# c976237222/HunyuanVideo_efficiency

Hardware: AMD Instinct MI355X
Metric: denoise-steps/sec (720x1280x129f, HunyuanVideo DiT 20+40 blocks, bf16) (higher is better)
Workload: dtype bf16

## Files before the change

hunyuanvideo_efficiency_amd/csrc/hv_attention.hip:

```cpp
#include "hv_attention.hpp"

using namespace hv_attn;

namespace {

constexpr int QTILE = 256;

__global__ __launch_bounds__(256) void attn_combine_kernel(const float* __restrict__ part_o, const float* __restrict__ part_ml,
                                                            bf16_t* __restrict__ o, int64_t so, int n_q, int n_heads, int n_splits) {
    const int64_t idx = (int64_t)blockIdx.x * blockDim.x + threadIdx.x;
    const int64_t total = (int64_t)n_q * n_heads * 32;
    if (idx >= total) return;
    const int d4 = (int)(idx & 31);
    const int64_t rh = idx >> 5;
    const int head = (int)(rh % n_heads);
    const int64_t row = rh / n_heads;
    float m = -INFINITY;
    for (int s = 0; s < n_splits; ++s) m = fmaxf(m, part_ml[(((int64_t)s * n_q + row) * n_heads + head) * 2]);
    float4 acc = make_float4(0.f, 0.f, 0.f, 0.f);
    float l = 0.f;
    for (int s = 0; s < n_splits; ++s) {
        const int64_t ri = ((int64_t)s * n_q + row) * n_heads + head;
        const float w = __builtin_amdgcn_exp2f(part_ml[ri * 2] - m);
        const float4 v = *reinterpret_cast<const float4*>(part_o + ri * D + d4 * 4);
        acc.x += v.x * w; acc.y += v.y * w; acc.z += v.z * w; acc.w += v.w * w;
        l += part_ml[ri * 2 + 1] * w;
    }
    const float inv = 1.0f / l;
    u32x2 w2;
    w2[0] = pack_bf2(acc.x * inv, acc.y * inv);
    w2[1] = pack_bf2(acc.z * inv, acc.w * inv);
    *reinterpret_cast<u32x2*>(o + row * so + head * D + d4 * 4) = w2;
}

int attn_launch(const AttnArgs& a, dim3 grid, hipStream_t stream) { return launch_w4(a, grid, stream); }

constexpr int KMAX_ROWS = 2048;
__global__ __launch_bounds__(256) void attn_kmax_kernel(const bf16_t* __restrict__ k, int64_t sk, int n_kv, unsigned* __restrict__ out) {
    __shared__ float wmax[4];
    const int head = blockIdx.y, t = threadIdx.x, ch = t & 15;
    const int r0 = blockIdx.x * KMAX_ROWS, r1 = min(r0 + KMAX_ROWS, n_kv);
    float best = 0.f;
    for (int row = r0 + (t >> 4); row < r1; row += 16) {
        const u32x4 w = *reinterpret_cast<const u32x4*>(k + (int64_t)row * sk + head * D + ch * 8);
        float s = 0.f;
#pragma unroll
        for (int j = 0; j < 4; ++j) {
            const float lo = bf2f_lo(w[j]), hi = bf2f_hi(w[j]);
            s += lo * lo + hi * hi;
        }
#pragma unroll
        for (int o = 8; o > 0; o >>= 1) s += __shfl_xor(s, o, 64);
        best = fmaxf(best, s);
    }
    best = fmaxf(best, __shfl_xor(best, 16, 64));
    best = fmaxf(best, __shfl_xor(best, 32, 64));
    if ((t & 63) == 0) wmax[t >> 6] = best;
    __syncthreads();
    if (t == 0) atomicMax(out + head, __float_as_uint(fmaxf(fmaxf(wmax[0], wmax[1]), fmaxf(wmax[2], wmax[3]))));
}

int attn_prepare_kmax(AttnArgs& a, void* workspace, int64_t workspace_bytes, hipStream_t stream) {
    a.kmax2 = nullptr;
    if (!workspace || workspace_bytes < KMAX_BYTES || a.n_heads > KMAX_HEADS || a.n_kv < 64 * KVT) return HV_OK;
    if (hipMemsetAsync(workspace, 0, KMAX_BYTES, stream) != hipSuccess) return HV_ERR_LAUNCH;
    attn_kmax_kernel<<<dim3((unsigned)((a.n_kv + KMAX_ROWS - 1) / KMAX_ROWS), (unsigned)a.n_heads), dim3(256), 0, stream>>>(a.k, a.sk, a.n_kv, (unsigned*)workspace);
    a.kmax2 = (const unsigned*)workspace;
    return HV_OK;
}

}

extern "C" int64_t hv_attn_workspace_bytes(int n_q, int n_kv, int n_heads) {
    (void)n_kv;
    return (int64_t)KMAX_BYTES + (int64_t)2 * n_q * n_heads * (128 + 2) * (int64_t)sizeof(float);
}

extern "C" int hv_attn_fwd_bf16(const void* q, const void* k, const void* v, void* o, int64_t stride_q, int64_t stride_k,
                                int64_t stride_v, int64_t stride_o, int n_q, int n_kv, int n_heads, int head_dim,
                                float scale, void* workspace, int64_t workspace_bytes, hipStream_t stream) {
    if (!q || !k || !v || !o || head_dim != D || n_heads <= 0 || n_q < 0 || n_kv < 0 || (stride_q & 7) || (stride_k & 7) ||
        (stride_v & 7) || (stride_o & 3))
        return HV_ERR_ARG;
    if (n_q == 0) return HV_OK;
    if (n_kv == 0) return HV_ERR_ARG;
    AttnArgs a;
    a.q = (const bf16_t*)q; a.k = (const bf16_t*)k; a.v = (const bf16_t*)v; a.o = (bf16_t*)o;
    a.sq = stride_q; a.sk = stride_k; a.sv = stride_v; a.so = stride_o;
    a.n_q = n_q; a.n_kv = n_kv; a.n_heads = n_heads;
    a.n_qtiles = (n_q + QTILE - 1) / QTILE;
    a.scale_log2e = scale * 1.4426950408889634f;
    a.n_splits = 1; a.split_keys = n_kv; a.part_o = nullptr; a.part_ml = nullptr; a.partial = 0;
    if (attn_prepare_kmax(a, workspace, workspace_bytes, stream) != HV_OK) return HV_ERR_LAUNCH;
    {
        const int64_t nwg = (int64_t)a.n_qtiles * n_heads;
        const int ntile = (n_kv + KVT - 1) / KVT;
        const double r1 = (double)((nwg + 255) / 256), r2 = 0.5 * (double)((2 * nwg + 255) / 256);
        if (workspace && ntile >= 64 && r2 < 0.97 * r1 && workspace_bytes >= hv_attn_workspace_bytes(n_q, n_kv, n_heads)) {
            a.n_splits = 2;
            a.split_keys = ((ntile + 1) / 2) * KVT;
            a.part_o = (float*)((char*)workspace + KMAX_BYTES);
            a.part_ml = a.part_o + (int64_t)2 * n_q * n_heads * D;
        }
    }
    if (attn_launch(a, dim3((unsigned)(a.n_qtiles * n_heads), (unsigned)a.n_splits), stream) != HV_OK) return HV_ERR_LAUNCH;
    if (a.n_splits > 1) {
        const int64_t total = (int64_t)n_q * n_heads * 32;
        attn_combine_kernel<<<dim3((unsigned)((total + 255) / 256)), dim3(256), 0, stream>>>(a.part_o, a.part_ml, a.o, a.so, n_q, n_heads,
                                                                                           a.n_splits);
    }
    return hv_check_launch();
}

extern "C" int hv_attn_partial_bf16(const void* q, const void* k, const void* v, int64_t stride_q, int64_t stride_k, int64_t stride_v,
                                    int n_q, int n_kv, int n_heads, int head_dim, float scale, void* part_o, void* part_ml,
                                    int n_slots, int slot, int splits, hipStream_t stream) {
    if (!q || !k || !v || !part_o || !part_ml || head_dim != D || n_heads <= 0 || n_q < 0 || n_kv <= 0 || (stride_q & 7) ||
        (stride_k & 7) || (stride_v & 7) || (splits != 1 && splits != 2) || slot < 0 || slot + splits > n_slots)
        return HV_ERR_ARG;
    if (n_q == 0) return HV_OK;
    const int ntile = (n_kv + KVT - 1) / KVT;
    if (splits == 2 && ntile < 2) return HV_ERR_ARG;
    AttnArgs a;
    a.q = (const bf16_t*)q; a.k = (const bf16_t*)k; a.v = (const bf16_t*)v; a.o = nullptr;
    a.sq = stride_q; a.sk = stride_k; a.sv = stride_v; a.so = 0;
    a.n_q = n_q; a.n_kv = n_kv; a.n_heads = n_heads;
    a.n_qtiles = (n_q + QTILE - 1) / QTILE;
    a.scale_log2e = scale * 1.4426950408889634f;
    a.n_splits = splits;
    a.split_keys = splits == 2 ? ((ntile + 1) / 2) * KVT : n_kv;
    a.part_o = (float*)part_o + (int64_t)slot * n_q * n_heads * D;
    a.part_ml = (float*)part_ml + (int64_t)slot * n_q * n_heads * 2;
    a.partial = 1;
    a.kmax2 = nullptr;
    if (attn_launch(a, dim3((unsigned)(a.n_qtiles * n_heads), (unsigned)splits), stream) != HV_OK) return HV_ERR_LAUNCH;
    return hv_check_launch();
}

extern "C" int hv_attn_merge_bf16(const void* part_o, const void* part_ml, void* o, int64_t stride_o, int n_q, int n_heads, int n_slots,
                                  hipStream_t stream) {
    if (!part_o || !part_ml || !o || n_heads <= 0 || n_q < 0 || n_slots <= 0 || (stride_o & 3)) return HV_ERR_ARG;
    if (n_q == 0) return HV_OK;
    const int64_t total = (int64_t)n_q * n_heads * 32;
    attn_combine_kernel<<<dim3((unsigned)((total + 255) / 256)), dim3(256), 0, stream>>>((const float*)part_o, (const float*)part_ml,
                                                                                       (bf16_t*)o, stride_o, n_q, n_heads, n_slots);
    return hv_check_launch();
}

extern "C" int hv_attn_suggest_splits(int n_q, int n_kv, int n_heads) {
    const int64_t nwg = (int64_t)((n_q + QTILE - 1) / QTILE) * n_heads;
    const int ntile = (n_kv + KVT - 1) / KVT;
    const double r1 = (double)((nwg + 255) / 256), r2 = 0.5 * (double)((2 * nwg + 255) / 256);
    return (ntile >= 64 && r2 < 0.97 * r1) ? 2 : 1;
}
```

hunyuanvideo_efficiency_amd/ops.py:

```python
from __future__ import annotations

from typing import Optional

import torch

from . import _lib

BF16 = torch.bfloat16
ACT_NONE, ACT_GELU_TANH, ACT_SILU = 0, 1, 2
PROFILE_ATTN = None


def _chk(t: torch.Tensor, dtype, name: str, last_contig: bool = True):
    if not t.is_cuda:
        raise _lib.HVKernelError(f"{name}: expected a GPU tensor (this package has no CPU path), got {t.device}")
    if t.dtype != dtype:
        raise TypeError(f"{name}: expected {dtype}, got {t.dtype}")
    if last_contig and t.dim() > 0 and t.stride(-1) != 1:
        raise ValueError(f"{name}: innermost dimension must be contiguous")


def _rows(t: torch.Tensor, name: str):
    if t.dim() == 1:
        return 1, t.shape[0], t.shape[0]
    d = t.shape[-1]
    n = t.numel() // d
    ld = t.stride(-2)
    exp = ld
    for i in range(t.dim() - 2, -1, -1):
        if t.shape[i] != 1 and t.stride(i) != exp:
            raise ValueError(f"{name}: rows are not uniformly strided {t.shape} {t.stride()}")
        exp *= t.shape[i]
    return n, d, ld


def ln_modulate(x, shift=None, scale=None, out=None, eps: float = 1e-6, affine: bool = False):
    _chk(x, BF16, "x")
    m, d, ldx = _rows(x, "x")
    if out is None:
        out = torch.empty(x.shape, dtype=BF16, device=x.device)
    _chk(out, BF16, "out")
    mo, do, ldo = _rows(out, "out")
    assert (mo, do) == (m, d)
    for t, n in ((shift, "shift"), (scale, "scale")):
        if t is not None:
            _chk(t, BF16, n)
            assert t.numel() == d and t.is_contiguous(), f"{n} must be a contiguous [{d}] vector (batch 1)"
    _lib.call("ln_modulate_bf16", x, shift, scale, out, m, d, ldx, ldo, eps,
                                               1 if affine else 0)
    return out


def qknorm_rope_(qkv, q_weight, k_weight, cos, sin, n_rope: int, n_heads: int, k_offset: int, eps: float = 1e-6, out=None):
    _chk(qkv, BF16, "qkv")
    n, _, ld = _rows(qkv, "qkv")
    _chk(q_weight, BF16, "q_weight"), _chk(k_weight, BF16, "k_weight")
    if n_rope > 0:
        _chk(cos, torch.float32, "cos"), _chk(sin, torch.float32, "sin")
        assert cos.is_contiguous() and sin.is_contiguous() and cos.shape[-1] == 128 and cos.shape[0] >= n_rope
    if out is not None:
        _chk(out, BF16, "out", False)
        assert out.dim() == 3 and out.shape[0] == n and out.stride(2) == 1 and out.shape[2] % 128 == 0
        assert out.shape[1] * out.shape[2] == 2 * n_heads * 128, (out.shape, n_heads)
        _lib.call("qknorm_rope_scatter_bf16", qkv, q_weight, k_weight, cos, sin, n, n_rope, n_heads, 128, ld, k_offset, eps,
                  out, out.stride(0), out.shape[2] // 128, out.stride(1))
        return out
    _lib.call("qknorm_rope_bf16", qkv, q_weight, k_weight, cos, sin, n,
                                               n_rope, n_heads, 128, ld, k_offset, eps)
    return qkv


def gemm(a, w, bias=None, out=None, act: int = ACT_NONE, n_split: int = 0, out1=None, act1: int = ACT_NONE,
         gate=None, res=None):
    _chk(a, BF16, "a"), _chk(w, BF16, "w")
    m, k, lda = _rows(a, "a")
    n, kw, ldw = _rows(w, "w")
    assert k == kw, (a.shape, w.shape)
    n0 = n_split if 0 < n_split < n else n
    if out is None:
        out = torch.empty(*a.shape[:-1], n0, dtype=BF16, device=a.device)
    _chk(out, BF16, "out")
    mo, no, ld0 = _rows(out, "out")
    assert mo == m and no >= n0
    ld1 = 0
    if n0 < n:
        _chk(out1, BF16, "out1")
        m1, n1, ld1 = _rows(out1, "out1")
        assert m1 == m and n1 >= n - n0
    for t, nm in ((bias, "bias"), (gate, "gate")):
        if t is not None:
            _chk(t, BF16, nm)
            assert t.numel() == n and t.is_contiguous()
    ld_res = 0
    if res is not None:
        _chk(res, BF16, "res")
        mr, nr, ld_res = _rows(res, "res")
        assert mr == m and nr == n
    _lib.call("gemm_bf16", a, lda, w, ldw, bias, m, n, k, out, ld0, act, n0,
                                        out1, ld1, act1, gate, res, ld_res)
    return out


def linear_smallm(x, w, bias=None, silu_in: bool = False, silu_out: bool = False, out=None, addend=None):
    _chk(x, BF16, "x"), _chk(w, BF16, "w")
    m, k, ldx = _rows(x, "x")
    n, kw, ldw = _rows(w, "w")
    assert k == kw and ldw == k and m <= 4
    if out is None:
        out = torch.empty(*x.shape[:-1], n, dtype=BF16, device=x.device)
    _, _, ldo = _rows(out, "out")
    if bias is not None:
        _chk(bias, BF16, "bias")
    if addend is not None:
        _chk(addend, BF16, "addend")
        assert addend.shape == out.shape and addend.stride() == out.stride()
    _lib.call("linear_smallm_bf16", x, w, bias, addend, out, m, n, k, ldx, ldo,
                                                 (1 if silu_in else 0) | (2 if silu_out else 0))
    return out


_attn_ws = {}


ATTN_MIN_WORKSPACE = 256


def _attn_workspace(n_q, n_kv, n_heads, device):
    if n_kv < 64 * 64:
        return None
    n_wg = ((n_q + 255) // 256) * n_heads
    need = ATTN_MIN_WORKSPACE if n_wg >= 16 * 256 else int(_lib.host("attn_workspace_bytes", n_q, n_kv, n_heads))
    key = str(device)
    ws = _attn_ws.get(key)
    if ws is None or ws.numel() < need:
        ws = torch.empty(need, dtype=torch.uint8, device=device)
        _attn_ws[key] = ws
    return ws


def attn_fwd(q, k, v, out, n_heads: int, scale: Optional[float] = None, kv_split_workspace: bool = True):
    for t, nm in ((q, "q"), (k, "k"), (v, "v"), (out, "out")):
        _chk(t, BF16, nm)
        assert t.dim() == 2
    n_q, n_kv = q.shape[0], k.shape[0]
    assert v.shape[0] == n_kv and out.shape[0] == n_q
    if scale is None:
        scale = 128 ** -0.5
    prof = PROFILE_ATTN
    if prof is not None:
        e0, e1 = torch.cuda.Event(enable_timing=True), torch.cuda.Event(enable_timing=True)
        e0.record()
    ws = _attn_workspace(n_q, n_kv, n_heads, q.device) if kv_split_workspace else None
    _lib.call("attn_fwd_bf16", q, k, v, out, q.stride(0), k.stride(0), v.stride(0),
                                            out.stride(0), n_q, n_kv, n_heads, 128, scale, ws,
                                            0 if ws is None else ws.numel())
    if prof is not None:
        e1.record()
        prof.append((e0, e1, n_q, n_kv, n_heads))
    return out


class AttnPartials:

    def __init__(self, n_slots: int, n_q: int, n_heads: int, device):
        self.n_slots, self.n_q, self.n_heads = n_slots, n_q, n_heads
        self.o = torch.empty(n_slots, n_q, n_heads, 128, dtype=torch.float32, device=device)
        self.ml = torch.empty(n_slots, n_q, n_heads, 2, dtype=torch.float32, device=device)
        self.used = 0


def attn_suggest_splits(n_q: int, n_kv: int, n_heads: int) -> int:
    return int(_lib.host("attn_suggest_splits", n_q, n_kv, n_heads))


def attn_partial(q, k, v, parts: AttnPartials, n_heads: int, splits: int = 1, scale: Optional[float] = None):
    for t, nm in ((q, "q"), (k, "k"), (v, "v")):
        _chk(t, BF16, nm)
        assert t.dim() == 2
    n_q, n_kv = q.shape[0], k.shape[0]
    assert v.shape[0] == n_kv and n_q == parts.n_q and n_heads == parts.n_heads and parts.used + splits <= parts.n_slots
    if scale is None:
        scale = 128 ** -0.5
    prof = PROFILE_ATTN
    if prof is not None:
        e0, e1 = torch.cuda.Event(enable_timing=True), torch.cuda.Event(enable_timing=True)
        e0.record()
    _lib.call("attn_partial_bf16", q, k, v, q.stride(0), k.stride(0), v.stride(0), n_q, n_kv, n_heads,
                                                128, scale, parts.o, parts.ml, parts.n_slots, parts.used, splits)
    if prof is not None:
        e1.record()
        prof.append((e0, e1, n_q, n_kv, n_heads))
    parts.used += splits


def attn_merge(parts: AttnPartials, out):
    _chk(out, BF16, "out")
    assert out.dim() == 2 and out.shape[0] == parts.n_q and parts.used >= 1
    _lib.call("attn_merge_bf16", parts.o, parts.ml, out, out.stride(0), parts.n_q, parts.n_heads,
                                              parts.used)
    return out


def patchify(x_f32, out=None):
    _chk(x_f32, torch.float32, "x")
    assert x_f32.is_contiguous() and x_f32.dim() == 4
    c, t, h, w = x_f32.shape
    if out is None:
        out = torch.empty(t * (h // 2) * (w // 2), c * 4, dtype=BF16, device=x_f32.device)
    _lib.call("patchify_f32_bf16", x_f32, out, c, t, h, w)
    return out


def unpatchify(y, c: int, t: int, h: int, w: int, out=None):
    _chk(y, BF16, "y")
    assert y.dim() == 2
    if out is None:
        out = torch.empty(c, t, h, w, dtype=BF16, device=y.device)
    _lib.call("unpatchify_bf16", y, out, c, t, h, w, y.stride(0))
    return out


def euler_step_(sample_f32, model_out_bf16, dt: float):
    _chk(sample_f32, torch.float32, "sample"), _chk(model_out_bf16, BF16, "model_out")
    assert sample_f32.is_contiguous() and model_out_bf16.is_contiguous() and sample_f32.numel() == model_out_bf16.numel()
    _lib.call("euler_step_f32", sample_f32, model_out_bf16, float(dt), sample_f32.numel())
    return sample_f32


def euler_step_f32_(sample_f32, model_out_f32, dt: float):
    _chk(sample_f32, torch.float32, "sample"), _chk(model_out_f32, torch.float32, "model_out")
    assert sample_f32.is_contiguous() and model_out_f32.is_contiguous() and sample_f32.numel() == model_out_f32.numel()
    _lib.call("euler_step_f32_f32", sample_f32, model_out_f32, float(dt), sample_f32.numel())
    return sample_f32


def masked_mean(x, mask_i32=None):
    _chk(x, BF16, "x")
    assert x.dim() == 2 and x.is_contiguous()
    out = torch.empty(x.shape[1], dtype=BF16, device=x.device)
    if mask_i32 is not None:
        _chk(mask_i32, torch.int32, "mask")
    _lib.call("masked_mean_bf16", x, mask_i32, out, x.shape[0], x.shape[1])
    return out


def broadcast_row_(src, dst):
    _chk(src, BF16, "src"), _chk(dst, BF16, "dst")
    assert dst.dim() == 2 and src.numel() == dst.shape[1]
    _lib.call("broadcast_row_bf16", src, dst, dst.shape[0], dst.shape[1], dst.stride(0))
    return dst


def timestep_embedding(t_f32, dim: int = 256, max_period: float = 10000.0):
    _chk(t_f32, torch.float32, "t")
    t_f32 = t_f32.reshape(-1).contiguous()
    out = torch.empty(t_f32.numel(), dim, dtype=BF16, device=t_f32.device)
    _lib.call("timestep_embedding_bf16", t_f32, out, t_f32.numel(), dim, max_period)
    return out


def fp8_dequant(w8, scale_bf16, out_bf16):
    if not w8.is_cuda or w8.dtype != torch.float8_e4m3fn:
        raise _lib.HVKernelError("fp8_dequant: expected a float8_e4m3fn GPU tensor")
    _chk(scale_bf16, BF16, "scale"), _chk(out_bf16, BF16, "out")
    assert w8.is_contiguous() and out_bf16.is_contiguous() and out_bf16.numel() == w8.numel()
    _lib.call("fp8_dequant_bf16", w8, scale_bf16, out_bf16, w8.numel())
    return out_bf16


FP8 = torch.float8_e4m3fn


def ln_modulate_fp8(x, shift=None, scale=None, out_q=None, out_scale=None, eps: float = 1e-6):
    _chk(x, BF16, "x")
    m, d, ldx = _rows(x, "x")
    if out_q is None:
        out_q = torch.empty(m, d, dtype=FP8, device=x.device)
    if out_scale is None:
        out_scale = torch.empty(m, dtype=torch.float32, device=x.device)
    assert out_q.dtype == FP8 and out_q.is_cuda and out_q.shape[-1] == d and out_q.stride(-1) == 1 and out_scale.numel() >= m
    for t, n in ((shift, "shift"), (scale, "scale")):
        if t is not None:
            _chk(t, BF16, n)
            assert t.numel() == d and t.is_contiguous()
    _lib.call("ln_modulate_fp8", x, shift, scale, out_q, out_scale, m, d, ldx, out_q.stride(-2) if out_q.dim() > 1 else d, eps)
    return out_q, out_scale


def quant_rows_fp8(x, out_q=None, out_scale=None):
    _chk(x, BF16, "x")
    m, k, ldx = _rows(x, "x")
    if out_q is None:
        out_q = torch.empty(m, k, dtype=FP8, device=x.device)
    if out_scale is None:
        out_scale = torch.empty(m, dtype=torch.float32, device=x.device)
    assert out_q.dtype == FP8 and out_q.is_cuda and out_q.shape[-1] == k and out_q.stride(-1) == 1 and out_scale.numel() >= m
    _lib.call("quant_rows_fp8", x, ldx, out_q, out_q.stride(-2) if out_q.dim() > 1 else k, out_scale, m, k)
    return out_q, out_scale


def gemm_fp8(a_q, a_scale, w_q, w_scale, bias=None, out=None, act: int = ACT_NONE, n_split: int = 0, out1=None,
             act1: int = ACT_NONE, gate=None, res=None):
    for t, nm in ((a_q, "a_q"), (w_q, "w_q")):
        if not t.is_cuda or t.dtype != FP8:
            raise _lib.HVKernelError(f"gemm_fp8: {nm} must be a float8_e4m3fn GPU tensor")
    _chk(a_scale, torch.float32, "a_scale"), _chk(w_scale, BF16, "w_scale")
    m, k, lda = _rows(a_q, "a_q")
    n, kw, ldw = _rows(w_q, "w_q")
    assert k == kw and a_scale.numel() >= m and w_scale.numel() == 1
    n0 = n_split if 0 < n_split < n else n
    if out is None:
        out = torch.empty(m, n0, dtype=BF16, device=a_q.device)
    _chk(out, BF16, "out")
    mo, no, ld0 = _rows(out, "out")
    assert mo == m and no >= n0
    ld1 = 0
    if n0 < n:
        _chk(out1, BF16, "out1")
        m1, n1, ld1 = _rows(out1, "out1")
        assert m1 == m and n1 >= n - n0
    for t, nm in ((bias, "bias"), (gate, "gate")):
        if t is not None:
            _chk(t, BF16, nm)
            assert t.numel() == n and t.is_contiguous()
    ld_res = 0
    if res is not None:
        _chk(res, BF16, "res")
        mr, nr, ld_res = _rows(res, "res")
        assert mr == m and nr == n
    _lib.call("gemm_fp8", a_q, lda, a_scale, w_q, ldw, w_scale, bias, m, n, k, out, ld0, act, n0, out1, ld1, act1, gate, res, ld_res)
    return out


def copy3d(src, dst, n_batch: int, rows: int, cols: int, src_bs: int, src_ld: int, dst_bs: int, dst_ld: int):
    _chk(src, BF16, "src", False), _chk(dst, BF16, "dst", False)
    _lib.call("copy3d_bf16", src, dst, n_batch, rows, cols, src_bs, src_ld, dst_bs, dst_ld)
    return dst
```

Baseline: 0.1188.

## Split only the tail wave of attention query tiles across KV chunks

Adds an attention launch planner. When the workgroup count does not fill a whole number of 256-wide waves, the planner runs the aligned bulk of query tiles unsplit and launches the leftover tail tiles with a KV split of up to 8 ways, then merges them with the combine kernel. This targets the partially filled last wave on the GPU at the cost of an extra launch, partial-result traffic and a combine pass. The Python side now always queries the planner for workspace size and keys the workspace by stream.

Result: no change. 0.1195 (median of 6 runs) (+0.5%).

```diff
diff --git a/hunyuanvideo_efficiency_amd/csrc/hv_attention.hip b/hunyuanvideo_efficiency_amd/csrc/hv_attention.hip
--- a/hunyuanvideo_efficiency_amd/csrc/hv_attention.hip
+++ b/hunyuanvideo_efficiency_amd/csrc/hv_attention.hip
@@ -69,11 +69,48 @@
     return HV_OK;
 }
 
+constexpr double TAIL_MIN_SAVING = 0.25;
+struct AttnPlan {
+    int splits = 1;
+    int q_whole = 0;
+    int tail_splits = 1;
+    int64_t part_bytes = 0;
+};
+AttnPlan attn_plan(int n_q, int n_kv, int n_heads) {
+    AttnPlan p;
+    const int n_qtiles = (n_q + QTILE - 1) / QTILE;
+    const int64_t nwg = (int64_t)n_qtiles * n_heads;
+    const int ntile = (n_kv + KVT - 1) / KVT;
+    if (ntile < 64) return p;
+    const double r1 = (double)((nwg + 255) / 256), r2 = 0.5 * (double)((2 * nwg + 255) / 256);
+    if (r2 < 0.97 * r1) {
+        p.splits = 2;
+        p.part_bytes = (int64_t)2 * n_q * n_heads * (D + 2) * (int64_t)sizeof(float);
+        return p;
+    }
+    if (nwg % 256 == 0) return p;
+    int g = 256;
+    while (n_heads % g) g >>= 1;
+    const int blk = 256 / g;
+    p.q_whole = (n_qtiles / blk) * blk;
+    if (p.q_whole == 0) return p;
+    const int64_t rest = (int64_t)(n_qtiles - p.q_whole) * n_heads;
+    double best = (double)((rest + 255) / 256);
+    const double whole = best;
+    for (int s = 2; s <= 8 && ntile >= 32 * s; ++s) {
+        const double t = (double)((rest * s + 255) / 256) / s;
+        if (t < best - 1e-9) { best = t; p.tail_splits = s; }
+    }
+    if (whole - best < TAIL_MIN_SAVING) p.tail_splits = 1;
+    if (p.tail_splits > 1)
+        p.part_bytes = (int64_t)p.tail_splits * (n_q - p.q_whole * QTILE) * n_heads * (D + 2) * (int64_t)sizeof(float);
+    return p;
+}
+
 }
 
 extern "C" int64_t hv_attn_workspace_bytes(int n_q, int n_kv, int n_heads) {
-    (void)n_kv;
-    return (int64_t)KMAX_BYTES + (int64_t)2 * n_q * n_heads * (128 + 2) * (int64_t)sizeof(float);
+    return (int64_t)KMAX_BYTES + attn_plan(n_q, n_kv, n_heads).part_bytes;
 }
 
 extern "C" int hv_attn_fwd_bf16(const void* q, const void* k, const void* v, void* o, int64_t stride_q, int64_t stride_k,
@@ -92,16 +129,35 @@
     a.scale_log2e = scale * 1.4426950408889634f;
     a.n_splits = 1; a.split_keys = n_kv; a.part_o = nullptr; a.part_ml = nullptr; a.partial = 0;
     if (attn_prepare_kmax(a, workspace, workspace_bytes, stream) != HV_OK) return HV_ERR_LAUNCH;
-    {
-        const int64_t nwg = (int64_t)a.n_qtiles * n_heads;
-        const int ntile = (n_kv + KVT - 1) / KVT;
-        const double r1 = (double)((nwg + 255) / 256), r2 = 0.5 * (double)((2 * nwg + 255) / 256);
-        if (workspace && ntile >= 64 && r2 < 0.97 * r1 && workspace_bytes >= hv_attn_workspace_bytes(n_q, n_kv, n_heads)) {
-            a.n_splits = 2;
-            a.split_keys = ((ntile + 1) / 2) * KVT;
-            a.part_o = (float*)((char*)workspace + KMAX_BYTES);
-            a.part_ml = a.part_o + (int64_t)2 * n_q * n_heads * D;
-        }
+    const AttnPlan p = attn_plan(n_q, n_kv, n_heads);
+    const bool use_split = workspace && p.part_bytes > 0 && workspace_bytes >= (int64_t)KMAX_BYTES + p.part_bytes;
+    const int ntile = (n_kv + KVT - 1) / KVT;
+    if (use_split && p.tail_splits > 1) {
+        const int rows0 = p.q_whole * QTILE, n_q2 = n_q - rows0;
+        AttnArgs a0 = a;
+        a0.n_q = rows0;
+        a0.n_qtiles = p.q_whole;
+        if (attn_launch(a0, dim3((unsigned)(a0.n_qtiles * n_heads), 1u), stream) != HV_OK) return HV_ERR_LAUNCH;
+        AttnArgs a1 = a;
+        a1.q += (int64_t)rows0 * a.sq;
+        a1.o = nullptr;
+        a1.n_q = n_q2;
+        a1.n_qtiles = (n_q2 + QTILE - 1) / QTILE;
+        a1.n_splits = p.tail_splits;
+        a1.split_keys = ((ntile + p.tail_splits - 1) / p.tail_splits) * KVT;
+        a1.part_o = (float*)((char*)workspace + KMAX_BYTES);
+        a1.part_ml = a1.part_o + (int64_t)p.tail_splits * n_q2 * n_heads * D;
+        if (attn_launch(a1, dim3((unsigned)(a1.n_qtiles * n_heads), (unsigned)a1.n_splits), stream) != HV_OK) return HV_ERR_LAUNCH;
+        const int64_t total = (int64_t)n_q2 * n_heads * 32;
+        attn_combine_kernel<<<dim3((unsigned)((total + 255) / 256)), dim3(256), 0, stream>>>(a1.part_o, a1.part_ml, a.o + (int64_t)rows0 * a.so,
+                                                                                           a.so, n_q2, n_heads, a1.n_splits);
+        return hv_check_launch();
+    }
+    if (use_split) {
+        a.n_splits = 2;
+        a.split_keys = ((ntile + 1) / 2) * KVT;
+        a.part_o = (float*)((char*)workspace + KMAX_BYTES);
+        a.part_ml = a.part_o + (int64_t)2 * n_q * n_heads * D;
     }
     if (attn_launch(a, dim3((unsigned)(a.n_qtiles * n_heads), (unsigned)a.n_splits), stream) != HV_OK) return HV_ERR_LAUNCH;
     if (a.n_splits > 1) {
diff --git a/hunyuanvideo_efficiency_amd/ops.py b/hunyuanvideo_efficiency_amd/ops.py
--- a/hunyuanvideo_efficiency_amd/ops.py
+++ b/hunyuanvideo_efficiency_amd/ops.py
@@ -128,9 +128,9 @@
 def _attn_workspace(n_q, n_kv, n_heads, device):
     if n_kv < 64 * 64:
         return None
-    n_wg = ((n_q + 255) // 256) * n_heads
-    need = ATTN_MIN_WORKSPACE if n_wg >= 16 * 256 else int(_lib.host("attn_workspace_bytes", n_q, n_kv, n_heads))
-    key = str(device)
+    need = int(_lib.host("attn_workspace_bytes", n_q, n_kv, n_heads))
+    stream = torch.cuda.current_stream(device)
+    key = str(device) if stream == torch.cuda.default_stream(device) else (str(device), stream.cuda_stream)
     ws = _attn_ws.get(key)
     if ws is None or ws.numel() < need:
         ws = torch.empty(need, dtype=torch.uint8, device=device)
```
